# IQTLabs/WITW

Measured on AMD Instinct MI355X. Metric: image-pairs/sec (embedding+similarity), higher is better.
Workload: dtype f32

## Files before the change

include/witw_hip.h:

```cpp
#ifndef WITW_HIP_H
#define WITW_HIP_H

#ifdef __cplusplus
extern "C" {
#endif

const char* witw_last_error(void);
int witw_version(void);
int witw_device_check(int device);
const char* witw_last_kernel_variant(void);
const char* witw_last_conv_form(void);


int witw_conv3x3_tile_n(int cout);
int witw_conv3x3_workgroup_waves(int B, int H, int W, int Cout, int stride_h);
long long witw_conv3x3_packed_floats(int cout, int cin);
int witw_conv3x3_bias_floats(int cout);
int witw_conv3x3_pack_weights(const float* w_kcrs, float* wpk, int cout, int cin, int transpose_flip, void* stream);
int witw_nchw_to_nhwc8(const float* x, float* y, int B, int C, int H, int W, void* stream);
int witw_conv3x3_fwd(const float* x, const float* wpk, const float* bias, const float* dropmask, float* y, int B, int H,
                     int W, int Cin, int Cout, int stride_h, int pad_circular, int relu, int pool, int out_nchw,
                     void* stream);

int witw_conv3x3_first_pack(const float* w, float* wf, int C, int round_bf16, void* stream);
int witw_conv_first2_bf16_fwd(const float* x, const void* wf0, const float* bias0, const void* wpk2, const float* bias2, void* y,
                              int B, int C, int H, int W, int pad_circular, void* stream);
int witw_conv_first2_bf16_fwd_train(const float* x, const void* wf0, const float* bias0, const void* wpk2, const float* bias2, void* y,
                                    unsigned char* pool_code, unsigned char* gate_bits, int B, int C, int H, int W, int pad_circular,
                                    void* stream);
int witw_conv3x3_bf16_gatebits_ok(int B, int H, int W, int Cin, int Cout);
int witw_conv3x3_bf16_fwd_gatebits(const void* x_bf16, const void* wpk_bf16, const float* bias, const void* gate_bits, void* y, int B, int H,
                                   int W, int Cin, int Cout, int pad_circular, int relu, void* stream);
int witw_conv3x3_first_fwd(const float* x, const float* wf, const float* bias, void* y, int B, int C, int H, int W,
                           int pad_circular, int relu, int out_bf16, void* stream);

int witw_conv3x3_fwd_ex(const float* x, const float* wpk, const float* bias, const float* dropmask, const float* gate,
                        const float* post_scale, const float* post_shift, float* y, unsigned char* pool_code, int B, int H,
                        int W, int Cin, int Cout, int stride_h, int pad_circular, int relu, float lrelu_slope, int pool,
                        int out_nchw, int dilate_h, void* stream);
int witw_conv3x3_dil_skip(int enable);
long long witw_conv3x3_packed_floats_wino(int cout, int cin);
int witw_conv3x3_pack_weights_wino(const float* w_kcrs, float* wpk_wino, int cout, int cin, void* stream);
int witw_conv3x3_fwd_wino(const float* x, const float* wpk, const float* wpk_wino, const float* bias, const float* dropmask,
                          const float* gate, const float* post_scale, const float* post_shift, float* y, unsigned char* pool_code,
                          int B, int H, int W, int Cin, int Cout, int stride_h, int pad_circular, int relu, float lrelu_slope,
                          int pool, int out_nchw, int dilate_h, void* stream);
int witw_conv3x3_wino(int enable);
int witw_conv3x3_wino_run(int enable);
int witw_maxpool2x2_bwd(const float* dy, const unsigned char* pool_code, float* dx, int B, int Hp, int Wp, int H, int W,
                        int C, void* stream);
int witw_nchw_to_nhwc(const float* x, float* y, int B, int C, int H, int W, int Cpad, void* stream);
int witw_conv3x3_wgrad_splits(int B, int Ho, int Wo, int Cin, int Cout);
long long witw_conv3x3_wgrad_workspace_floats(int B, int H, int W, int Cin, int Cout, int stride_h);
int witw_conv3x3_wgrad(const float* x, const float* dz, float* dw, float* db, float* workspace, int B, int H, int W, int Cin,
                       int cin_real, int Cout, int stride_h, int pad_circular, int accumulate, void* stream);
int witw_adam_step(float* param, const float* grad, float* exp_avg, float* exp_avg_sq, long long n, float lr, float beta1,
                   float beta2, float eps, int step, void* stream);
int witw_adam_step_multi(float* const* param, const float* const* grad, float* const* exp_avg, float* const* exp_avg_sq,
                         const long long* n, const int* step, int count, float lr, float beta1, float beta2, float eps, void* stream);

long long witw_match_workspace_floats(int Bo, int Bs);
int witw_match_fwd(const float* ov, const float* su, int Bo, int Bs, int We, long long* orientation, float* distance,
                   float* score, float* workspace, void* stream);
int witw_match_fwd_masked(const float* ov, const float* su, int Bo, int Bs, int We, long long* orientation, float* distance,
                          float* score, float* workspace, const unsigned long long* shift_mask, void* stream);
long long witw_match_fixed_workspace_floats(int Bo, int Bs);
int witw_match_fwd_fixed(const float* ov, const float* su, int Bo, int Bs, int We, const long long* shift ,
                         long long* orientation, float* distance, float* score, float* workspace, void* stream);
long long witw_match_spectrum_floats(long long n_embeddings);
int witw_match_spectrum(const float* emb, float* spec, int B, int W, int role ,
                        void* stream);
long long witw_match_dft_workspace_floats(int Bo, int Bs);
int witw_match_fwd_dft(const float* ov, const float* su, const float* spec_ov, const float* spec_su, int Bo, int Bs, int We,
                       long long* orientation, float* distance, float* score, float* workspace, void* stream);
int witw_match_fwd_dft_gap(const float* ov, const float* su, const float* spec_ov, const float* spec_su, int Bo, int Bs, int We,
                           long long* orientation, float* distance, float* score, float* gap, float* workspace, void* stream);
int witw_match_fwd_dft_masked(const float* ov, const float* su, const float* spec_ov, const float* spec_su, int Bo, int Bs, int We,
                              long long* orientation, float* distance, float* score, float* gap , float* workspace,
                              const unsigned long long* shift_mask, void* stream);
long long witw_match_bwd_scratch_floats(int Bo, int Bs, int We);
int witw_match_bwd(const float* ov, const float* su, const long long* orientation, const float* score, const float* workspace,
                   const float* grad_distance, float* grad_ov, float* grad_su, float* scratch, int Bo, int Bs, int We,
                   void* stream);
int witw_crop_overhead(const float* ov, const long long* orientation, float* out , int Bo, int Bs,
                       int We, void* stream);
int witw_l2_distance(const float* cropped , const float* su , float* distance, int Bo, int Bs, int n,
                     void* stream);
int witw_rank_count(const float* distance , int* ranks , int Bo, int Bs, int true_offset, void* stream);

int witw_topk_smallest(const float* distance, float* values, long long* indices, int Bo, int Bs, int k, long long row_offset,
                       void* stream);
long long witw_topk_workspace_bytes(int Bo, int Bs, int k);
int witw_topk_smallest_ws(const float* distance, float* values, long long* indices, int Bo, int Bs, int k, long long row_offset,
                          void* workspace, void* stream);
int witw_topk_smallest_after(const float* distance, float* values, long long* indices, int Bo, int Bs, int k, long long row_offset,
                             const float* after_value, const long long* after_index, void* workspace, void* stream);
int witw_rank_count_thresh(const float* distance, const float* threshold, int* ranks, int Bo, int Bs, void* stream);

int witw_match_pairs(const float* ov, const float* su, const float* wn, const float* sn, const int* pair_o, const int* pair_s,
                     int n_pairs, int Bo, int Bs, int We, long long* orientation, float* distance, float* score, void* stream);
int witw_rank_count_band(const float* distance, const float* threshold, float eps, int* counts, int* pair_o, int* pair_s,
// ... 204 lines not shown
```

witw_amd/_lib.py:

```python
import ctypes
import os
from ctypes import c_char_p, c_float, c_int, c_longlong, c_void_p

from . import build as _build

_LIB = None
_GUARDS = None

SIGNATURES = {
    'witw_last_error': (c_char_p, []),
    'witw_version': (c_int, []),
    'witw_last_kernel_variant': (c_char_p, []),
    'witw_last_conv_form': (c_char_p, []),
    'witw_device_check': (c_int, [c_int]),
    'witw_conv3x3_tile_n': (c_int, [c_int]),
    'witw_conv3x3_workgroup_waves': (c_int, [c_int] * 5),
    'witw_conv3x3_packed_floats': (c_longlong, [c_int, c_int]),
    'witw_conv3x3_bias_floats': (c_int, [c_int]),
    'witw_conv3x3_pack_weights': (c_int, [c_void_p, c_void_p, c_int, c_int, c_int, c_void_p]),
    'witw_nchw_to_nhwc8': (c_int, [c_void_p, c_void_p, c_int, c_int, c_int, c_int, c_void_p]),
    'witw_conv3x3_fwd': (c_int, [c_void_p, c_void_p, c_void_p, c_void_p, c_void_p] + [c_int] * 10 + [c_void_p]),
    'witw_conv3x3_fwd_ex': (c_int, [c_void_p] * 9 + [c_int] * 8 + [c_float] + [c_int] * 3 + [c_void_p]),
    'witw_conv3x3_dil_skip': (c_int, [c_int]),
    'witw_conv3x3_packed_floats_wino': (c_longlong, [c_int, c_int]),
    'witw_conv3x3_pack_weights_wino': (c_int, [c_void_p, c_void_p, c_int, c_int, c_void_p]),
    'witw_conv3x3_fwd_wino': (c_int, [c_void_p] * 10 + [c_int] * 8 + [c_float] + [c_int] * 3 + [c_void_p]),
    'witw_conv3x3_wino': (c_int, [c_int]),
    'witw_conv3x3_wino_run': (c_int, [c_int]),
    'witw_maxpool2x2_bwd': (c_int, [c_void_p, c_void_p, c_void_p] + [c_int] * 6 + [c_void_p]),
    'witw_conv3x3_packed_floats_taps4': (c_longlong, [c_int, c_int]),
    'witw_conv3x3_pack_weights_taps4': (c_int, [c_void_p, c_void_p, c_int, c_int, c_int, c_void_p]),
    'witw_conv3x3_fwd_taps4': (c_int, [c_void_p] * 7 + [c_int] * 6 + [c_float, c_int, c_void_p]),
    'witw_conv3x3_taps4_ksplit': (c_int, [c_int] * 5),
    'witw_conv3x3_fwd_taps4_ex': (c_int, [c_void_p] * 7 + [c_int] * 6 + [c_float] + [c_int] * 5 + [c_void_p]),
    'witw_conv3x3_wgrad_taps4': (c_int, [c_void_p] * 5 + [c_int] * 7 + [c_void_p]),
    'witw_nchw_to_nhwc': (c_int, [c_void_p, c_void_p, c_int, c_int, c_int, c_int, c_int, c_void_p]),
    'witw_conv3x3_wgrad_splits': (c_int, [c_int] * 5),
    'witw_conv3x3_wgrad_workspace_floats': (c_longlong, [c_int] * 6),
    'witw_conv3x3_wgrad': (c_int, [c_void_p] * 5 + [c_int] * 9 + [c_void_p]),
    'witw_adam_step': (c_int, [c_void_p, c_void_p, c_void_p, c_void_p, c_longlong, c_float, c_float, c_float, c_float, c_int,
                               c_void_p]),
    'witw_adam_step_multi': (c_int, [c_void_p] * 6 + [c_int, c_float, c_float, c_float, c_float, c_void_p]),
    'witw_conv3x3_first_pack': (c_int, [c_void_p, c_void_p, c_int, c_int, c_void_p]),
    'witw_conv3x3_first_fwd': (c_int, [c_void_p, c_void_p, c_void_p, c_void_p] + [c_int] * 7 + [c_void_p]),
    'witw_conv3x3_bf16_mfma16': (c_int, [c_int]),
    'witw_conv3x3_bf16_wres': (c_int, [c_int]),
    'witw_conv3x3_bf16_packed_elems': (c_longlong, [c_int, c_int]),
    'witw_conv3x3_bf16_pack_weights': (c_int, [c_void_p, c_void_p, c_int, c_int, c_void_p]),
    'witw_conv3x3_bf16_pack_weights_ex': (c_int, [c_void_p, c_void_p, c_int, c_int, c_int, c_void_p]),
    'witw_conv3x3_bf16_pack_weights_multi': (c_int, [c_void_p] * 7 + [c_int, c_void_p]),
    'witw_nchw_f32_to_nhwc_bf16': (c_int, [c_void_p, c_void_p] + [c_int] * 5 + [c_void_p]),
    'witw_conv3x3_bf16_fwd': (c_int, [c_void_p] * 4 + [c_int] * 10 + [c_void_p]),
    'witw_conv3x3_bf16_fwd_ex': (c_int, [c_void_p] * 7 + [c_int] * 11 + [c_void_p]),
    'witw_maxpool2x2_bwd_bf16': (c_int, [c_void_p] * 3 + [c_int] * 6 + [c_void_p]),
    'witw_octet_elems': (c_longlong, [c_int] * 4),
    'witw_nhwc_bf16_to_octet': (c_int, [c_void_p, c_void_p] + [c_int] * 4 + [c_void_p]),
    'witw_conv3x3_wgrad_bf16_workspace_floats': (c_longlong, [c_int] * 6),
    'witw_conv3x3_wgrad_bf16': (c_int, [c_void_p] * 5 + [c_int] * 9 + [c_void_p]),
    'witw_conv3x3_wgrad_bf16_nhwc_workspace_floats': (c_longlong, [c_int] * 6),
    'witw_conv3x3_wgrad_bf16_mfma16': (c_int, [c_int]),
    'witw_conv3x3_wgrad_bf16_nhwc': (c_int, [c_void_p] * 5 + [c_int] * 9 + [c_void_p]),
    'witw_conv3x3_f16x3_packed_elems': (c_longlong, [c_int, c_int]),
    'witw_conv3x3_f16x3_pack_weights': (c_int, [c_void_p, c_void_p, c_int, c_int, c_void_p]),
    'witw_nchw_f32_to_split_f16': (c_int, [c_void_p, c_void_p] + [c_int] * 5 + [c_void_p]),
    'witw_split_f16_to_f32': (c_int, [c_void_p, c_void_p, c_longlong, c_int, c_void_p]),
    'witw_conv3x3_f16x3_fwd': (c_int, [c_void_p] * 4 + [c_int] * 10 + [c_void_p]),
    'witw_conv3x3_f16x3_pack_weights_ex': (c_int, [c_void_p, c_void_p, c_int, c_int, c_int, c_void_p]),
    'witw_conv3x3_f16x3_fwd_ex': (c_int, [c_void_p] * 8 + [c_int] * 11 + [c_void_p]),
    'witw_maxpool2x2_bwd_split': (c_int, [c_void_p] * 3 + [c_int] * 6 + [c_void_p]),
    'witw_octet_split_elems': (c_longlong, [c_int] * 4),
    'witw_split_f16_to_octet': (c_int, [c_void_p, c_void_p] + [c_int] * 4 + [c_void_p]),
    'witw_conv3x3_wgrad_f16x3_workspace_floats': (c_longlong, [c_int] * 6),
    'witw_conv3x3_wgrad_f16x3': (c_int, [c_void_p] * 6 + [c_int] * 9 + [c_void_p]),
    'witw_conv4x4s2_first_fwd': (c_int, [c_void_p] * 6 + [c_int] * 5 + [c_float, c_void_p]),
    'witw_conv4x4s2_first_fwd_bf16': (c_int, [c_void_p] * 6 + [c_int] * 5 + [c_float, c_void_p]),
    'witw_conv3x3_bf16_packed_elems_taps4': (c_longlong, [c_int, c_int]),
    'witw_conv3x3_bf16_pack_weights_taps4': (c_int, [c_void_p, c_void_p, c_int, c_int, c_void_p]),
    'witw_conv3x3_bf16_fwd_taps4': (c_int, [c_void_p] * 6 + [c_int] * 5 + [c_float] + [c_int] * 3 + [c_void_p]),
    'witw_conv3x3_bf16_taps4_ksplit': (c_int, [c_int] * 5),
    'witw_conv3x3_bf16_fwd_taps4_splitk': (c_int, [c_void_p] * 3 + [c_int] * 6 + [c_void_p]),
    'witw_space_to_depth2_mosaic_bf16': (c_int, [c_void_p, c_void_p] + [c_int] * 5 + [c_void_p]),
# ... 148 lines not shown
```

witw_amd/csrc/conv3x3.hip:

```cpp
#include "common.h"
#include <stdlib.h>
#include <algorithm>

namespace {

constexpr int TW_WIDE = 64;

__device__ const f32x4 g_zero_f4[1] = {{0.f, 0.f, 0.f, 0.f}};

struct ConvArgs {
    const float* x;
    const float* wpk;
    const float* bias;
    const float* dropmask;
    const float* post_scale;
    const float* post_shift;
    float lrelu;
    unsigned char* pool_code;
    const float* gate;
    float* y;
    int B, H, W, Cin, Cout;
    int Ho, Wo;
    int tiles_x, tiles_y;
    int n_tiles, sp_total, sp_per_xcd, xcd_map;
    int circ, relu, out_nchw;
    int force_nw;
    int force_geo;
    int dil_h;
    int tap_base;
    int ksplit, kc_per_split;
    size_t split_stride;
    int s2d, s2d_h, s2d_w, valid_h, valid_w;
    int wino;
    const float* wpk_wino;
    int wino_items, wino_wgs;
#ifdef WITW_STAMPS
    unsigned long long* stamps;
#endif
};

template <int NW, bool POOL>
__device__ __forceinline__ void conv_wino_h2(const ConvArgs& p, f32x4* smem) {
    constexpr int TH = NW, TW = 64, IW = TW + 2, IH = TH + 2;
    constexpr int NTHREADS = 64 * NW;
    constexpr int WTN = 64;
    constexpr int IN_F4 = 2 * IH * IW;
    constexpr int W_F4 = 12 * 2 * WTN;
    constexpr int STAGE_F4 = IN_F4 + W_F4;
    constexpr int NIN = (IN_F4 + NTHREADS - 1) / NTHREADS;
    constexpr int NWT = W_F4 / NTHREADS;
    static_assert(NWT * NTHREADS == W_F4, "the filter slab splits evenly over the workgroup");

    int tid = threadIdx.x;
    asm volatile("" : "+v"(tid));
    const int lane = tid & 63;
    const int wave = tid >> 6;
    const int l31 = lane & 31;
    const int hq = lane >> 5;

    const int tiles_img = p.tiles_x * p.tiles_y;
    auto item_sp = [&](int it, int& ntile) {
        if (p.xcd_map) {
            const int g = it >> 3;
            ntile = g % p.n_tiles;
            return (it & 7) * p.sp_per_xcd + g / p.n_tiles;
        }
        ntile = it / p.sp_total;
        return it - ntile * p.sp_total;
    };
    auto step_item = [&](int it) { return p.wino_items - it > p.wino_wgs ? it + p.wino_wgs : p.wino_items; };
    auto next_item = [&](int it) {
        int nt;
        while (it < p.wino_items && item_sp(it, nt) >= p.sp_total) it = step_item(it);
        return it;
    };
    int it = next_item(blockIdx.x);
    if (it >= p.wino_items) return;
    const int nkc = p.Cin >> 3;

    constexpr unsigned OOR = 0x80000000u;
    const size_t img_floats = (size_t)p.H * p.W * p.Cin;
    int ntile, b, oy0, ox0;
    __amdgpu_buffer_rsrc_t in_rs, w_rs;
    unsigned gin[NIN];
    auto decode = [&](int item, int& nt_, int& b_, int& oy0_, int& ox0_) {
        int sp = item_sp(item, nt_);
        b_ = sp / tiles_img;
        sp -= b_ * tiles_img;
        const int ty = sp / p.tiles_x;
        oy0_ = ty * TH;
        ox0_ = (sp - ty * p.tiles_x) * TW;
    };
    auto stage_from = [&](int nt_, int b_, int oy0_, int ox0_, bool live) {
        in_rs = __builtin_amdgcn_make_buffer_rsrc((void*)(p.x + (size_t)b_ * img_floats), 0, live ? (unsigned)(img_floats * 4) : 0u,
                                                  0x00020000);
        w_rs = __builtin_amdgcn_make_buffer_rsrc((void*)(reinterpret_cast<const f32x4*>(p.wpk_wino) + (size_t)nt_ * nkc * W_F4), 0,
                                                 live ? (unsigned)nkc * W_F4 * 16u : 0u, 0x00020000);
        if (!live) return;
        int t = tid;
        asm volatile("" : "+v"(t));
#pragma unroll
        for (int i = 0; i < NIN; ++i) {
            const int s = t + i * NTHREADS;
            const int pix = s >> 1, q = s & 1;
            const int r = pix / IW, c = pix - r * IW;
            const int gr = oy0_ - 1 + r;
            int gc = ox0_ - 1 + c;
            bool ok = (s < IN_F4) && gr >= 0 && gr < p.H;
            if (p.circ) {
                gc %= p.W;
                if (gc < 0) gc += p.W;
            } else {
                ok = ok && gc >= 0 && gc < p.W;
            }
            gin[i] = ok ? (unsigned)((((size_t)gr * p.W + gc) * p.Cin + q * 4) * 4) : OOR;
        }
    };
    decode(it, ntile, b, oy0, ox0);
    stage_from(ntile, b, oy0, ox0, true);
    const unsigned gwoff = (unsigned)tid * 16u;
    f32x4 rin[NIN], rw[NWT];
    auto load_one = [&](int kc, int i) {
        if (i < NIN) rin[i] = __builtin_bit_cast(f32x4, __builtin_amdgcn_raw_buffer_load_b128(in_rs, gin[i], (unsigned)kc * 32u, 0));
        else rw[i - NIN] = __builtin_bit_cast(f32x4, __builtin_amdgcn_raw_buffer_load_b128(
                 w_rs, gwoff, (unsigned)kc * W_F4 * 16u + (unsigned)(i - NIN) * (NTHREADS * 16u), 0));
    };
    auto store_one = [&](int buf, int i) {
        f32x4* in_s = smem + buf * STAGE_F4;
        if (i < NIN) {
            const int s = tid + i * NTHREADS;
            f32x4* dst = (NIN * NTHREADS == IN_F4 || s < IN_F4) ? in_s + (s & 1) * (IH * IW) + (s >> 1) : smem + 2 * STAGE_F4;
            *dst = rin[i];
        } else {
            in_s[IN_F4 + tid + (i - NIN) * NTHREADS] = rw[i - NIN];
        }
    };

    const int wm = wave >> 1, wn = wave & 1;
    const int abase = hq * (IH * IW) + 2 * wm * IW + l31;
    const int wbase = hq * WTN + wn * 32 + l31;
    f32x16 acc[4][2];
#pragma unroll
    for (int t = 0; t < 4; ++t)
#pragma unroll
        for (int ct = 0; ct < 2; ++ct)
#pragma unroll
            for (int r = 0; r < 16; ++r) acc[t][ct][r] = 0.f;

    f32x4 fa[2][4], fb[2][4];
    auto read_a = [&](int set, const f32x4* in_s, int s, int i) { fa[set][i] = in_s[abase + i * IW + 32 * (s & 1) + (s >> 1)]; };
    auto read_b = [&](int set, const f32x4* w_s, int kw, int t) { fb[set][t] = w_s[(kw * 4 + t) * 2 * WTN + wbase]; };
    auto transform2 = [&](int set, int k) {
        const int j = k >> 1;
        const float d0 = fa[set][0][j], d1 = fa[set][1][j], d2 = fa[set][2][j], d3 = fa[set][3][j];
        if ((k & 1) == 0) {
            fa[set][0][j] = d0 - d2;
            fa[set][3][j] = d1 - d3;
        } else {
            fa[set][1][j] = d1 + d2;
            fa[set][2][j] = d2 - d1;
        }
    };
    auto mfma_one = [&](int set, int bset, int ct, int i) {
        const int j = i >> 2, t = i & 3;
        acc[t][ct] = __builtin_amdgcn_mfma_f32_32x32x2f32(fa[set][t][j], fb[bset][t][j], acc[t][ct], 0, 0, 0);
    };

#pragma unroll
    for (int i = 0; i < NIN + NWT; ++i) load_one(0, i);
#pragma unroll
    for (int i = 0; i < NIN + NWT; ++i) store_one(0, i);
    __syncthreads();
#pragma unroll
    for (int i = 0; i < 4; ++i) read_b(0, smem + IN_F4, 0, i);
    __builtin_amdgcn_sched_barrier(0);
#pragma unroll
    for (int i = 0; i < 4; ++i) read_a(0, smem, 0, i);
#pragma unroll
    for (int k = 0; k < 8; ++k) transform2(0, k);

    auto step = [&](int set, int bset, int ct, auto&& mem, bool barrier_mid) {
#pragma unroll
        for (int i = 0; i < 16; ++i) {
            mfma_one(set, bset, ct, i);
            mem(i);
            if (i >= 8) transform2(set ^ 1, i - 8);
            __builtin_amdgcn_sched_barrier(0);
            if (barrier_mid && i == 7) {
                __syncthreads();
                __builtin_amdgcn_sched_barrier(0);
            }
        }
    };
    static_assert(16 - 6 - (NIN + NWT) >= 0, "step too short to hide the staging instructions");

    auto chunk = [&](int cur, int kn) __attribute__((always_inline)) {
        const f32x4* in_s = smem + cur * STAGE_F4;
        const f32x4* w_s = in_s + IN_F4;
        const f32x4* in_n = smem + (cur ^ 1) * STAGE_F4;
        step(0, 0, 0, [&](int i) {
            if (i < 4) read_a(1, in_s, 1, i);
            else if (i < 6) read_b(1, w_s, 1, i - 4);
            else if (i < 6 + NIN + NWT) load_one(kn, i - 6);
        }, false);
        step(1, 0, 1, [&](int i) {
            if (i < 4) read_a(0, in_s, 2, i);
            else if (i < 6) read_b(1, w_s, 1, i - 2);
        }, false);
        step(0, 1, 0, [&](int i) {
            if (i < 4) read_a(1, in_s, 3, i);
            else if (i < 8) read_b(0, w_s, 2, i - 4);
        }, false);
        step(1, 1, 1, [&](int i) {
            if (i < 4) read_a(0, in_s, 4, i);
            else if (i < 4 + NIN + NWT) store_one(cur ^ 1, i - 4);
        }, false);
        step(0, 0, 0, [&](int i) {
            if (i < 4) read_a(1, in_s, 5, i);
        }, true);
        step(1, 0, 1, [&](int i) {
            if (i < 4) read_a(0, in_n, 0, i);
            else if (i < 8) read_b(1, in_n + IN_F4, 0, i - 4);
        }, false);
#pragma unroll
        for (int t = 0; t < 4; ++t) fb[0][t] = fb[1][t];
    };

    const int Hy = POOL ? (p.Ho >> 1) : p.Ho;
    const int Wy = POOL ? (p.Wo >> 1) : p.Wo;
    float* slab = reinterpret_cast<float*>(smem + 2 * STAGE_F4 + 1) + wave * (32 * 32);
    const int prow = lane >> 3, pc4 = (lane & 7) * 4;
    int cur = 0;
    for (;;) {
        for (int kc = 1; kc < nkc; ++kc) {
            chunk(cur, kc);
            cur ^= 1;
        }
        const int it_n = next_item(step_item(it));
        const bool more = it_n < p.wino_items;
        int ntile_n = ntile, b_n = b, oy0_n = oy0, ox0_n = ox0;
        if (more) decode(it_n, ntile_n, b_n, oy0_n, ox0_n);
        stage_from(ntile_n, b_n, oy0_n, ox0_n, more);
        chunk(cur, 0);
        cur ^= 1;

        const int n0 = ntile * WTN;
        f32x16 yv[2][2];
#pragma unroll
        for (int ct = 0; ct < 2; ++ct)
#pragma unroll
            for (int r = 0; r < 16; ++r) {
                const float m0 = acc[0][ct][r], m1 = acc[1][ct][r], m2 = acc[2][ct][r], m3 = acc[3][ct][r];
                yv[0][ct][r] = (m0 + m1) + m2;
                yv[1][ct][r] = (m1 - m2) - m3;
            }
        const int nb = n0 + wn * 32;
        const int nch = nb + l31;
        const float bv = p.bias[nch];
        const float dm = (p.dropmask != nullptr && nch < p.Cout) ? p.dropmask[(size_t)b * p.Cout + nch] : 1.f;
        const int act = p.relu;
        auto fin = [&](float v) {
            v = (v + bv) * dm;
            if (act == 1) v = fmaxf(v, 0.f);
            else if (act == 2) v = v > 0.f ? v : v * p.lrelu;
            return v;
        };
        if constexpr (!POOL) {
#pragma unroll
            for (int k = 0; k < 2; ++k)
#pragma unroll
                for (int ct = 0; ct < 2; ++ct) {
#pragma unroll
                    for (int r = 0; r < 16; ++r) slab[((r & 3) + 8 * (r >> 2) + 4 * hq) * 32 + l31] = fin(yv[k][ct][r]);
                    const int yy = oy0 + 2 * wm + k;
#pragma unroll
// ... 19 lines not shown
                        const int pc = 16 * ct + 4 * g + 2 * hq + e;
                        slab[pc * 32 + l31] = fin(m);
                        const int xx = (ox0 >> 1) + pc;
                        if (p.pool_code != nullptr && yy < Hy && xx < Wy && nch < p.Cout) {
                            const int code = (a00 == m) ? 0 : (a01 == m) ? 1 : (a10 == m) ? 2 : 3;
                            p.pool_code[(((size_t)b * Hy + yy) * Wy + xx) * p.Cout + nch] = (unsigned char)code;
                        }
                    }
#pragma unroll
            for (int g = 0; g < 4; ++g) {
                const int pc = g * 8 + prow;
                const f32x4 v = *reinterpret_cast<const f32x4*>(slab + pc * 32 + pc4);
                const int xx = (ox0 >> 1) + pc;
                if (yy < Hy && xx < Wy && nb + pc4 < p.Cout)
                    __builtin_nontemporal_store(v, reinterpret_cast<f32x4*>(p.y + (((size_t)b * Hy + yy) * Wy + xx) * p.Cout + nb + pc4));
            }
        }
        if (!more) break;
        it = it_n;
        ntile = ntile_n;
        b = b_n;
        oy0 = oy0_n;
        ox0 = ox0_n;
#pragma unroll
        for (int t = 0; t < 4; ++t)
#pragma unroll
            for (int ct = 0; ct < 2; ++ct)
#pragma unroll
                for (int r = 0; r < 16; ++r) acc[t][ct][r] = 0.f;
    }
}

template <int TN, int SH, bool POOL, int NW, int GEO, int TAPS = 9>
__global__ __launch_bounds__(64 * NW) void conv3x3_nhwc_f32_kernel(ConvArgs p) {
    static_assert(TAPS == 9 || TAPS == 4, "3x3 window or a 2x2 sub-window");
    constexpr bool NARROW = GEO == 1;
    constexpr bool DIL = GEO == 2;
    static_assert(!DIL || (TN == 128 && NW == 8 && SH == 1 && TAPS == 9 && !POOL), "the dilated form exists for the 8-wave 128-channel tile");
    constexpr int TH = NARROW ? 4 * NW : NW;
    constexpr int TW = NARROW ? 16 : 64;
    constexpr int IW = TW + 2;
    constexpr int NTHREADS = 64 * NW;
    constexpr int IH = (TH - 1) * SH + 3;
    constexpr int IN_F4 = 2 * IH * IW;
    constexpr int W_F4 = TAPS * 2 * TN;
    constexpr int STAGE_F4 = IN_F4 + W_F4;
    constexpr int NIN = (IN_F4 + NTHREADS - 1) / NTHREADS;
    constexpr int NWT = (W_F4 + NTHREADS - 1) / NTHREADS;
    constexpr int WGM = (TN == 128) ? NW / 2 : NW;
    constexpr int WM = (2 * NW) / WGM;
    constexpr int WN = 2;

    constexpr bool WINO = SH == 1 && TAPS == 9 && GEO == 0 && (TN == 128 || POOL);
    constexpr int WINO_F4 = WINO ? 2 * (2 * (NW + 2) * IW + 12 * 2 * 64) + 1 + NW * 256 : 0;
    constexpr int DIRECT_F4 = (2 * STAGE_F4 + 1 > NW * 512) ? 2 * STAGE_F4 + 1 : NW * 512;
    constexpr int SMEM_F4 = DIRECT_F4 > WINO_F4 ? DIRECT_F4 : WINO_F4;
    __shared__ f32x4 smem[SMEM_F4];
    static_assert(SMEM_F4 * 16 >= NW * 32 * 64 * 4, "the buffer must hold one epilogue slab per wave");
    if constexpr (WINO) {
        if (__builtin_expect(p.wino != 0, 0)) {
            conv_wino_h2<NW, POOL>(p, smem);
            return;
        }
    }

    const int tid = threadIdx.x;
    const int lane = tid & 63;
    const int wave = tid >> 6;
    const int l31 = lane & 31;
    const int hq = lane >> 5;

    int ntile, sp;
    if (p.xcd_map) {
        const int g = blockIdx.x >> 3;
        ntile = g % p.n_tiles;
        sp = (blockIdx.x & 7) * p.sp_per_xcd + g / p.n_tiles;
        if (sp >= p.sp_total) return;
    } else {
        ntile = blockIdx.x / p.sp_total;
        sp = blockIdx.x - ntile * p.sp_total;
    }
    const int tiles_img = p.tiles_x * p.tiles_y;
    const int b = sp / tiles_img;
    sp -= b * tiles_img;
    const int ty = sp / p.tiles_x;
    const int tx = sp - ty * p.tiles_x;
    const int oy0 = ty * TH;
    const int ox0 = tx * TW;
    const int n0 = ntile * TN;
    int nkc = p.Cin >> 3;
    int kc_lo = 0;
    if constexpr (TAPS == 4) {
        if (p.ksplit > 1) {
            kc_lo = (int)blockIdx.y * p.kc_per_split;
            nkc = min(nkc - kc_lo, p.kc_per_split);
        }
    }

    constexpr unsigned OOR = 0x80000000u;
    const int Hp = p.dil_h ? (p.H - 1) / 2 + 1 : p.H;
    const size_t img_floats = (size_t)Hp * p.W * p.Cin;
    __amdgpu_buffer_rsrc_t in_rs = __builtin_amdgcn_make_buffer_rsrc(
        (void*)(p.x + (size_t)b * img_floats + (size_t)kc_lo * 8), 0, (unsigned)(img_floats * 4) - (unsigned)kc_lo * 32u, 0x00020000);
    const unsigned wtile_bytes = (unsigned)nkc * W_F4 * 16u;
    __amdgpu_buffer_rsrc_t w_rs = __builtin_amdgcn_make_buffer_rsrc(
        (void*)(reinterpret_cast<const f32x4*>(p.wpk) + ((size_t)ntile * (p.Cin >> 3) + kc_lo) * W_F4), 0, wtile_bytes, 0x00020000);
    unsigned gin[NIN];
#pragma unroll
    for (int i = 0; i < NIN; ++i) {
        const int s = tid + i * NTHREADS;
        const int pix = s >> 1, q = s & 1;
        const int r = pix / IW, c = pix - r * IW;
        const int gr = oy0 * SH - 1 + r;
        int gc = ox0 - 1 + c;
// ... 420 lines not shown
    }
    reinterpret_cast<f32x4*>(wpk)[idx] = v;
}

__global__ void pack_weights_wino_kernel(const float* __restrict__ w, float* __restrict__ wpk, int Cout, int Cin, int nkc,
                                         size_t total) {
    const size_t idx = (size_t)blockIdx.x * blockDim.x + threadIdx.x;
    if (idx >= total) return;
    size_t t = idx;
    const int n = t % 64; t /= 64;
    const int q = t % 2; t /= 2;
    const int tr = t % 4; t /= 4;
    const int kw = t % 3; t /= 3;
    const int kc = t % nkc; t /= nkc;
    const int co = (int)t * 64 + n;
    f32x4 v = {0.f, 0.f, 0.f, 0.f};
#pragma unroll
    for (int j = 0; j < 4; ++j) {
        const int ci = kc * 8 + q * 4 + j;
        if (co < Cout && ci < Cin) {
            const float* g = w + ((size_t)co * Cin + ci) * 9 + kw;
            const float g0 = g[0], g1 = g[3], g2 = g[6];
            v[j] = tr == 0 ? g0 : tr == 1 ? ((g0 + g1) + g2) * 0.5f : tr == 2 ? ((g0 - g1) + g2) * 0.5f : g2;
        }
    }
    reinterpret_cast<f32x4*>(wpk)[idx] = v;
}

__global__ void nchw_to_nhwc8_kernel(const float* __restrict__ x, float* __restrict__ y, int B, int C, int H, int W) {
    const size_t npix = (size_t)B * H * W;
    const size_t idx = (size_t)blockIdx.x * blockDim.x + threadIdx.x;
    if (idx >= npix) return;
    const size_t hw = (size_t)H * W;
    const size_t b = idx / hw, r = idx - b * hw;
    float v[8];
#pragma unroll
    for (int c = 0; c < 8; ++c) v[c] = (c < C) ? x[(b * C + c) * hw + r] : 0.f;
    f32x4* o = reinterpret_cast<f32x4*>(y + idx * 8);
    o[0] = f32x4{v[0], v[1], v[2], v[3]};
    o[1] = f32x4{v[4], v[5], v[6], v[7]};
}

__global__ void nchw_to_nhwc_kernel(const float* __restrict__ x, float* __restrict__ y, int C, int Cp, size_t hw, size_t total) {
    const size_t idx = (size_t)blockIdx.x * blockDim.x + threadIdx.x;
    if (idx >= total) return;
    const int c = idx % Cp;
    const size_t t = idx / Cp;
    const size_t b = t / hw, r = t - b * hw;
    y[idx] = (c < C) ? x[(b * C + c) * hw + r] : 0.f;
}

int env_int(const char* name, int dflt);
int wino_run();

template <int TN, int SH, bool POOL, int NW, int GEO, int TAPS = 9>
int launch_conv_nw(ConvArgs a, hipStream_t st) {
    a.tiles_y = cdiv(a.Ho, GEO == 1 ? 4 * NW : NW);
    a.tiles_x = cdiv(a.Wo, GEO == 1 ? 16 : 64);
    const long long sp_total = (long long)a.B * a.tiles_x * a.tiles_y;
    a.n_tiles = cdiv(a.Cout, a.wino ? 64 : TN);
    a.sp_per_xcd = (int)((sp_total + 7) / 8);
    if (sp_total < 8) a.xcd_map = 0;
    const long long grid = a.xcd_map ? 8LL * a.sp_per_xcd * a.n_tiles : sp_total * a.n_tiles;
    if (grid <= 0 || grid > 0x7fffffffLL || sp_total > 0x7fffffffLL) {
        witw_set_error("conv3x3: grid %lld out of range", grid);
        return WITW_ERR_INVALID;
    }
    a.sp_total = (int)sp_total;
    const unsigned gy = (TAPS == 4 && a.ksplit > 1) ? (unsigned)a.ksplit : 1u;
    a.wino_items = (int)grid;
    a.wino_wgs = (int)grid;
    if (a.wino && wino_run()) {
        const int forced = env_int("WITW_CONV_WINO_WGS", 0);
        a.wino_wgs = (int)std::min<long long>(grid, forced > 0 ? forced : witw_cu_count());
    }
    hipLaunchKernelGGL((conv3x3_nhwc_f32_kernel<TN, SH, POOL, NW, GEO, TAPS>), dim3(a.wino ? (unsigned)a.wino_wgs : (unsigned)grid, gy),
                       dim3(64 * NW), 0, st, a);
    WITW_CHECK_LAUNCH("conv3x3_nhwc_f32");
    witw_note_variant("conv3x3_nhwc_f32_kernel<%d,%d,%s,%d,%d,%d>", TN, SH, POOL ? "true" : "false", NW, GEO, TAPS);
    if (a.wino) witw_note_conv_form("wino_h2");
    return WITW_OK;
}

int choose_waves(int B, int Ho, int Wo, int Cout, int force_nw) {
    const int TN = (Cout >= 128) ? 128 : 64;
    const long long big = (long long)cdiv(Cout, TN) * B * cdiv(Wo, TW_WIDE) * cdiv(Ho, 8);
    if (force_nw == 4) return 4;
    return (force_nw == 8 || ((Ho % 8) == 0 && witw_fills_rounds(big))) ? 8 : 4;
}

bool choose_narrow(int Wo, int force_geo) { return force_geo == 1 || (force_geo != 0 && Wo <= 32); }

int env_int(const char* name, int dflt) {
    const char* e = getenv(name);
    return e ? atoi(e) : dflt;
}

int g_dil_skip = -1;
int dil_skip() {
    if (g_dil_skip < 0) {
        const char* e = getenv("WITW_CONV_DILSKIP");
        g_dil_skip = e ? (atoi(e) != 0) : 1;
    }
    return g_dil_skip;
}

int g_wino = -1;
int wino_on() {
    if (g_wino < 0) {
        const char* e = getenv("WITW_CONV_WINO");
        g_wino = e ? (atoi(e) != 0) : 1;
    }
    return g_wino;
}

int g_wino_run = -1;
int wino_run() {
    if (g_wino_run < 0) {
        const char* e = getenv("WITW_CONV_WINO_RUN");
        g_wino_run = e ? (atoi(e) != 0) : 1;
    }
    return g_wino_run;
}

template <int TN, int SH, bool POOL>
int launch_conv(ConvArgs a, hipStream_t st) {
    const bool wino = SH == 1 && (TN == 128 || POOL) && a.wpk_wino != nullptr && wino_on() && a.gate == nullptr && !a.dil_h &&
                      !a.out_nchw && a.post_scale == nullptr && (a.Cout & 3) == 0 && a.force_geo != 1 &&
                      !choose_narrow(a.Wo, a.force_geo);
    a.wino = wino ? 1 : 0;
    if (wino) return choose_waves(a.B, a.Ho, a.Wo, a.Cout, a.force_nw) == 8 ? launch_conv_nw<TN, SH, POOL, 8, 0>(a, st)
                                                                          : launch_conv_nw<TN, SH, POOL, 4, 0>(a, st);
#ifndef WITW_NO_NARROW
    if (choose_narrow(a.Wo, a.force_geo)) return launch_conv_nw<TN, SH, POOL, 4, 1>(a, st);
#endif
    if (choose_waves(a.B, a.Ho, a.Wo, a.Cout, a.force_nw) == 8) {
        if constexpr (TN == 128 && SH == 1 && !POOL) {
            if (a.dil_h && dil_skip()) return launch_conv_nw<TN, SH, POOL, 8, 2>(a, st);
        }
        return launch_conv_nw<TN, SH, POOL, 8, 0>(a, st);
    }
    return launch_conv_nw<TN, SH, POOL, 4, 0>(a, st);
}

template <int TN>
int launch_conv_taps4(const ConvArgs& a, hipStream_t st) {
#ifndef WITW_NO_NARROW
    if (choose_narrow(a.Wo, a.force_geo)) return launch_conv_nw<TN, 1, false, 4, 1, 4>(a, st);
#endif
    if (choose_waves(a.B, a.Ho, a.Wo, a.Cout, a.force_nw) == 8) return launch_conv_nw<TN, 1, false, 8, 0, 4>(a, st);
    return launch_conv_nw<TN, 1, false, 4, 0, 4>(a, st);
}

}

#ifdef WITW_STAMPS
unsigned long long* witw_conv_stamps_ptr = nullptr;
#endif

extern "C" {

int witw_conv3x3_tile_n(int cout) { return cout >= 128 ? 128 : 64; }

int witw_conv3x3_workgroup_waves(int B, int H, int W, int Cout, int stride_h) {
    if (B <= 0 || H <= 0 || W <= 0 || Cout <= 0 || (stride_h != 1 && stride_h != 2)) return -1;
    if (choose_narrow(W, env_int("WITW_CONV_GEO", -1))) return 4;
    return choose_waves(B, (H + 2 - 3) / stride_h + 1, W, Cout, env_int("WITW_CONV_NW", 0));
}

long long witw_conv3x3_packed_floats(int cout, int cin) {
    if (cout <= 0 || cin <= 0) return -1;
    const int TN = witw_conv3x3_tile_n(cout);
    const long long n_tiles = cdiv(cout, TN), nkc = cdiv(cin, 8);
    return n_tiles * nkc * 9 * 2 * TN * 4;
}
// ... 159 lines not shown
    a.tiles_y = 0;
    a.force_nw = env_int("WITW_CONV_NW", 0);
    a.force_geo = env_int("WITW_CONV_GEO", -1);
    a.xcd_map = env_int("WITW_CONV_XCD", 1) != 0;
    a.circ = pad_circular; a.relu = relu; a.out_nchw = out_nchw; a.dil_h = dilate_h; a.tap_base = 0;
    a.ksplit = 1; a.kc_per_split = 0; a.split_stride = 0; a.s2d = 0; a.s2d_h = a.s2d_w = a.valid_h = a.valid_w = 0;
    a.wino = 0; a.wpk_wino = wpk_wino;
#ifdef WITW_STAMPS
    a.stamps = witw_conv_stamps_ptr;
#endif
    hipStream_t st = (hipStream_t)stream;
    const int TN = witw_conv3x3_tile_n(Cout);
    if (TN == 128) {
        if (stride_h == 2) return launch_conv<128, 2, false>(a, st);
        return pool ? launch_conv<128, 1, true>(a, st) : launch_conv<128, 1, false>(a, st);
    }
    if (stride_h == 2) return launch_conv<64, 2, false>(a, st);
    return pool ? launch_conv<64, 1, true>(a, st) : launch_conv<64, 1, false>(a, st);
}

}

extern "C" {

int witw_conv3x3_fwd_ex(const float* x, const float* wpk, const float* bias, const float* dropmask, const float* gate,
                        const float* post_scale, const float* post_shift, float* y, unsigned char* pool_code, int B, int H,
                        int W, int Cin, int Cout, int stride_h, int pad_circular, int relu, float lrelu_slope, int pool,
                        int out_nchw, int dilate_h, void* stream) {
    return conv3x3_fwd_any(x, wpk, nullptr, bias, dropmask, gate, post_scale, post_shift, y, pool_code, B, H, W, Cin, Cout,
                           stride_h, pad_circular, relu, lrelu_slope, pool, out_nchw, dilate_h, stream);
}

int witw_conv3x3_fwd_wino(const float* x, const float* wpk, const float* wpk_wino, const float* bias, const float* dropmask,
                          const float* gate, const float* post_scale, const float* post_shift, float* y, unsigned char* pool_code,
                          int B, int H, int W, int Cin, int Cout, int stride_h, int pad_circular, int relu, float lrelu_slope,
                          int pool, int out_nchw, int dilate_h, void* stream) {
    WITW_CHECK_ARG(wpk_wino, "conv3x3_fwd_wino: null Winograd filter");
    return conv3x3_fwd_any(x, wpk, wpk_wino, bias, dropmask, gate, post_scale, post_shift, y, pool_code, B, H, W, Cin, Cout,
                           stride_h, pad_circular, relu, lrelu_slope, pool, out_nchw, dilate_h, stream);
}

int witw_conv3x3_wino(int enable) {
    const int prev = wino_on();
    if (enable >= 0) g_wino = enable != 0;
    return prev;
}

int witw_conv3x3_wino_run(int enable) {
    const int prev = wino_run();
    if (enable >= 0) g_wino_run = enable != 0;
    return prev;
}

long long witw_conv3x3_packed_floats_wino(int cout, int cin) {
    if (cout <= 0 || cin <= 0) return -1;
    return (long long)cdiv(cout, 64) * cdiv(cin, 8) * 12 * 2 * 64 * 4;
}

int witw_conv3x3_pack_weights_wino(const float* w_kcrs, float* wpk_wino, int cout, int cin, void* stream) {
    WITW_CHECK_ARG(w_kcrs && wpk_wino, "pack_weights_wino: null pointer");
    WITW_CHECK_ARG(cout > 0 && cin > 0, "pack_weights_wino: bad shape cout=%d cin=%d", cout, cin);
    const int n_tiles = cdiv(cout, 64), nkc = cdiv(cin, 8);
    const size_t total = (size_t)n_tiles * nkc * 12 * 2 * 64;
    hipLaunchKernelGGL(pack_weights_wino_kernel, dim3((unsigned)((total + 255) / 256)), dim3(256), 0, (hipStream_t)stream,
                       w_kcrs, wpk_wino, cout, cin, nkc, total);
    WITW_CHECK_LAUNCH("pack_weights_wino");
    return WITW_OK;
}

int witw_conv3x3_dil_skip(int enable) {
    const int prev = dil_skip();
    if (enable >= 0) g_dil_skip = enable != 0;
    return prev;
}

int witw_conv3x3_fwd(const float* x, const float* wpk, const float* bias, const float* dropmask, float* y, int B, int H,
                     int W, int Cin, int Cout, int stride_h, int pad_circular, int relu, int pool, int out_nchw,
                     void* stream) {
    return witw_conv3x3_fwd_ex(x, wpk, bias, dropmask, nullptr, nullptr, nullptr, y, nullptr, B, H, W, Cin, Cout, stride_h,
                               pad_circular, relu ? 1 : 0, 0.f, pool, out_nchw, 0, stream);
}

}
```

witw_amd/ops.py:

```python
import torch

from . import _lib


PROFILE = None
PROFILE_BY_KERNEL = None


def _stream():
    return torch.cuda.current_stream().cuda_stream


def _dev_f32(t, name):
    if not (isinstance(t, torch.Tensor) and t.is_cuda):
        raise _lib.WitwError('%s must be a CUDA(HIP) tensor: the WITW hot path has no CPU fallback' % name)
    if t.dtype != torch.float32:
        raise _lib.WitwError('%s must be float32, got %s' % (name, t.dtype))
    if not t.is_contiguous():
        raise _lib.WitwError('%s must be contiguous' % name)
    return t


def _p(t):
    return 0 if t is None else t.data_ptr()
# ... 1215 lines not shown

def gem_pool(x_nhwc, valid_hw, out, col0, p=3., scale=None, shift=None):
    lib = _lib.load()
    x = _dev_f32(x_nhwc, 'x')
    B, Hp, Wp, C = x.shape
    H, W = valid_hw
    _lib.check(lib.witw_gem_pool(x.data_ptr(), out.data_ptr(), B, Hp, Wp, H, W, C, out.shape[1], col0, float(p), _p(scale),
                                 _p(shift), _stream()), 'witw_gem_pool')
    return out


def embed_normalize_(f):
    lib = _lib.load()
    f = _dev_f32(f, 'f')
    _lib.check(lib.witw_embed_normalize(f.data_ptr(), f.shape[0], f.shape[1], _stream()), 'witw_embed_normalize')
    return f


def pairwise_sqdist(a, b, take_sqrt=False):
    lib = _lib.load()
    a, b = _dev_f32(a, 'a'), _dev_f32(b, 'b')
    if a.dim() != 2 or b.dim() != 2 or a.shape[1] != b.shape[1]:
        raise _lib.WitwError('pairwise_sqdist: need [Na,n] and [Nb,n]')
    D = torch.empty((a.shape[0], b.shape[0]), dtype=torch.float32, device=a.device)
    _lib.check(lib.witw_pairwise_sqdist(a.data_ptr(), b.data_ptr(), D.data_ptr(), a.shape[0], b.shape[0], a.shape[1],
                                        int(take_sqrt), _stream()), 'witw_pairwise_sqdist')
    return D


def exhaustive_triplet_loss(D, soft_margin=False, alpha=10., margin=1.):
    lib = _lib.load()
    D = _dev_f32(D, 'D')
    B = D.shape[0]
    loss = torch.empty((1,), dtype=torch.float32, device=D.device)
    ws = torch.empty((B,), dtype=torch.float32, device=D.device)
    _lib.check(lib.witw_exhaustive_triplet_loss(D.data_ptr(), B, int(soft_margin), float(alpha), float(margin),
                                                loss.data_ptr(), ws.data_ptr(), _stream()), 'witw_exhaustive_triplet_loss')
    return loss.reshape(())


def last_conv_form():
    v = _lib.load().witw_last_conv_form()
    return v.decode() if v else ''


def conv_wino(enable=None):
    return bool(_lib.load().witw_conv3x3_wino(-1 if enable is None else int(bool(enable))))


def conv_wino_run(enable=None):
    return bool(_lib.load().witw_conv3x3_wino_run(-1 if enable is None else int(bool(enable))))


def last_kernel_variant():
    v = _lib.load().witw_last_kernel_variant()
    return v.decode() if v else ''


def bf16_mfma16(enable=None):
    return bool(_lib.load().witw_conv3x3_bf16_mfma16(-1 if enable is None else int(bool(enable))))


def bf16_wres(enable=None):
    return bool(_lib.load().witw_conv3x3_bf16_wres(-1 if enable is None else int(bool(enable))))


class PackedConvBf16(_Packed):
    CPAD, DTYPE = 16, torch.bfloat16

    def __init__(self, weight, bias, transpose_flip=False, reuse=None):
        lib = _lib.load()
        w, reuse = self._filter_buffer(weight, transpose_flip, reuse, lib.witw_conv3x3_bf16_packed_elems)
        _lib.check(lib.witw_conv3x3_bf16_pack_weights_ex(w.data_ptr(), self.wpk.data_ptr(), self.cout, self.cin,
                                                         int(bool(transpose_flip)), _stream()), 'witw_conv3x3_bf16_pack_weights_ex')
        self._bias_buffer(reuse, bias)

    @classmethod
    def batch(cls, items):
        import ctypes
        lib = _lib.load()
        out, tab = [], []
        for weight, bias, transpose_flip, reuse in items:
            pk = cls.__new__(cls)
            w, reuse = pk._filter_buffer(weight, transpose_flip, reuse, lib.witw_conv3x3_bf16_packed_elems)
            pk._bias_buffer(reuse)
            b = None if bias is None else _dev_f32(bias.detach(), 'bias')
            if b is not None and b.numel() != pk.cout:
                raise _lib.WitwError('PackedConvBf16.batch: bias of %d elements for %d output channels' % (b.numel(), pk.cout))
            tab.append((w, pk.wpk, b, pk.bias, pk.cout, pk.cin, int(bool(transpose_flip))))
            out.append(pk)
        k = len(tab)
        if k:
            vp = ctypes.c_void_p
            _lib.check(lib.witw_conv3x3_bf16_pack_weights_multi(
                (vp * k)(*[t[0].data_ptr() for t in tab]), (vp * k)(*[t[1].data_ptr() for t in tab]),
                (vp * k)(*[None if t[2] is None else t[2].data_ptr() for t in tab]), (vp * k)(*[t[3].data_ptr() for t in tab]),
                (ctypes.c_int * k)(*[t[4] for t in tab]), (ctypes.c_int * k)(*[t[5] for t in tab]),
                (ctypes.c_int * k)(*[t[6] for t in tab]), k, _stream()), 'witw_conv3x3_bf16_pack_weights_multi')
        return out


def nchw_to_nhwc_bf16(x, cpad=16):
    lib = _lib.load()
    x = _dev_f32(x, 'x')
    B, C, H, W = x.shape
    y = torch.empty((B, H, W, cpad), dtype=torch.bfloat16, device=x.device)
# ... 291 lines not shown
```

Baseline: 2530.

## Stage Winograd conv inputs and filters via direct global-to-LDS buffer loads

Adds a DMA variant of the Winograd conv kernel that uses buffer loads writing straight into LDS instead of loading into registers and then storing to shared memory. The next chunk's transfers are spread over the MFMA steps, with a vmcnt wait before the mid barrier. The input staging layout is padded and reordered, plane-major instead of interleaved, to suit wave-contiguous LDS writes. It is on by default behind an env toggle. This saves registers and VALU/LDS store instructions, but it changes the LDS layout and how synchronisation is ordered.

```diff
diff --git a/include/witw_hip.h b/include/witw_hip.h
--- a/include/witw_hip.h
+++ b/include/witw_hip.h
@@ -47,6 +47,7 @@
                           int pool, int out_nchw, int dilate_h, void* stream);
 int witw_conv3x3_wino(int enable);
 int witw_conv3x3_wino_run(int enable);
+int witw_conv3x3_wino_dma(int enable);
 int witw_maxpool2x2_bwd(const float* dy, const unsigned char* pool_code, float* dx, int B, int Hp, int Wp, int H, int W,
                         int C, void* stream);
 int witw_nchw_to_nhwc(const float* x, float* y, int B, int C, int H, int W, int Cpad, void* stream);
diff --git a/witw_amd/_lib.py b/witw_amd/_lib.py
--- a/witw_amd/_lib.py
+++ b/witw_amd/_lib.py
@@ -27,6 +27,7 @@
     'witw_conv3x3_fwd_wino': (c_int, [c_void_p] * 10 + [c_int] * 8 + [c_float] + [c_int] * 3 + [c_void_p]),
     'witw_conv3x3_wino': (c_int, [c_int]),
     'witw_conv3x3_wino_run': (c_int, [c_int]),
+    'witw_conv3x3_wino_dma': (c_int, [c_int]),
     'witw_maxpool2x2_bwd': (c_int, [c_void_p, c_void_p, c_void_p] + [c_int] * 6 + [c_void_p]),
     'witw_conv3x3_packed_floats_taps4': (c_longlong, [c_int, c_int]),
     'witw_conv3x3_pack_weights_taps4': (c_int, [c_void_p, c_void_p, c_int, c_int, c_int, c_void_p]),
diff --git a/witw_amd/csrc/conv3x3.hip b/witw_amd/csrc/conv3x3.hip
--- a/witw_amd/csrc/conv3x3.hip
+++ b/witw_amd/csrc/conv3x3.hip
@@ -1,4 +1,5 @@
 #include "common.h"
+#include "lds_frag.h"
 #include <stdlib.h>
 #include <algorithm>
 
@@ -34,21 +35,23 @@
     int wino;
     const float* wpk_wino;
     int wino_items, wino_wgs;
+    int wino_dma;
 #ifdef WITW_STAMPS
     unsigned long long* stamps;
 #endif
 };
 
-template <int NW, bool POOL>
+template <int NW, bool POOL, bool DMA>
 __device__ __forceinline__ void conv_wino_h2(const ConvArgs& p, f32x4* smem) {
     constexpr int TH = NW, TW = 64, IW = TW + 2, IH = TH + 2;
     constexpr int NTHREADS = 64 * NW;
     constexpr int WTN = 64;
     constexpr int IN_F4 = 2 * IH * IW;
     constexpr int W_F4 = 12 * 2 * WTN;
-    constexpr int STAGE_F4 = IN_F4 + W_F4;
     constexpr int NIN = (IN_F4 + NTHREADS - 1) / NTHREADS;
     constexpr int NWT = W_F4 / NTHREADS;
+    constexpr int IN_PAD = NIN * NTHREADS;
+    constexpr int STAGE_F4 = IN_PAD + W_F4;
     static_assert(NWT * NTHREADS == W_F4, "the filter slab splits evenly over the workgroup");
 
     int tid = threadIdx.x;
@@ -82,6 +85,7 @@
     const size_t img_floats = (size_t)p.H * p.W * p.Cin;
     int ntile, b, oy0, ox0;
     __amdgpu_buffer_rsrc_t in_rs, w_rs;
+    i32x4 in_rd, w_rd;
     unsigned gin[NIN];
     auto decode = [&](int item, int& nt_, int& b_, int& oy0_, int& ox0_) {
         int sp = item_sp(item, nt_);
@@ -92,17 +96,24 @@
         ox0_ = (sp - ty * p.tiles_x) * TW;
     };
     auto stage_from = [&](int nt_, int b_, int oy0_, int ox0_, bool live) {
-        in_rs = __builtin_amdgcn_make_buffer_rsrc((void*)(p.x + (size_t)b_ * img_floats), 0, live ? (unsigned)(img_floats * 4) : 0u,
-                                                  0x00020000);
-        w_rs = __builtin_amdgcn_make_buffer_rsrc((void*)(reinterpret_cast<const f32x4*>(p.wpk_wino) + (size_t)nt_ * nkc * W_F4), 0,
-                                                 live ? (unsigned)nkc * W_F4 * 16u : 0u, 0x00020000);
+        const float* in_base = p.x + (size_t)b_ * img_floats;
+        const f32x4* w_base = reinterpret_cast<const f32x4*>(p.wpk_wino) + (size_t)nt_ * nkc * W_F4;
+        const unsigned in_bytes = live ? (unsigned)(img_floats * 4) : 0u, w_bytes = live ? (unsigned)nkc * W_F4 * 16u : 0u;
+        if constexpr (DMA) {
+            in_rd = raw_rsrc(in_base, in_bytes);
+            w_rd = raw_rsrc(w_base, w_bytes);
+        } else {
+            in_rs = __builtin_amdgcn_make_buffer_rsrc((void*)in_base, 0, in_bytes, 0x00020000);
+            w_rs = __builtin_amdgcn_make_buffer_rsrc((void*)w_base, 0, w_bytes, 0x00020000);
+        }
         if (!live) return;
         int t = tid;
         asm volatile("" : "+v"(t));
 #pragma unroll
         for (int i = 0; i < NIN; ++i) {
             const int s = t + i * NTHREADS;
-            const int pix = s >> 1, q = s & 1;
+            const int q = DMA ? (s >= IH * IW) : (s & 1);
+            const int pix = DMA ? s - q * (IH * IW) : s >> 1;
             const int r = pix / IW, c = pix - r * IW;
             const int gr = oy0_ - 1 + r;
             int gc = ox0_ - 1 + c;
@@ -119,6 +130,14 @@
     decode(it, ntile, b, oy0, ox0);
     stage_from(ntile, b, oy0, ox0, true);
     const unsigned gwoff = (unsigned)tid * 16u;
+    const unsigned smem_lds = (unsigned)__builtin_amdgcn_readfirstlane((int)lds_address(smem));
+    const unsigned wave_lds = (unsigned)__builtin_amdgcn_readfirstlane(wave) * 1024u;
+    auto dma_one = [&](int buf, int kc, int i) {
+        const unsigned st = smem_lds + (unsigned)buf * (STAGE_F4 * 16u) + wave_lds;
+        if (i < NIN) dma16(in_rd, st + (unsigned)i * (NTHREADS * 16u), gin[i], (unsigned)kc * 32u);
+        else dma16(w_rd, st + (unsigned)(IN_PAD + (i - NIN) * NTHREADS) * 16u, gwoff,
+                   (unsigned)kc * W_F4 * 16u + (unsigned)(i - NIN) * (NTHREADS * 16u));
+    };
     f32x4 rin[NIN], rw[NWT];
     auto load_one = [&](int kc, int i) {
         if (i < NIN) rin[i] = __builtin_bit_cast(f32x4, __builtin_amdgcn_raw_buffer_load_b128(in_rs, gin[i], (unsigned)kc * 32u, 0));
@@ -132,7 +151,7 @@
             f32x4* dst = (NIN * NTHREADS == IN_F4 || s < IN_F4) ? in_s + (s & 1) * (IH * IW) + (s >> 1) : smem + 2 * STAGE_F4;
             *dst = rin[i];
         } else {
-            in_s[IN_F4 + tid + (i - NIN) * NTHREADS] = rw[i - NIN];
+            in_s[IN_PAD + tid + (i - NIN) * NTHREADS] = rw[i - NIN];
         }
     };
 
@@ -166,13 +185,19 @@
         acc[t][ct] = __builtin_amdgcn_mfma_f32_32x32x2f32(fa[set][t][j], fb[bset][t][j], acc[t][ct], 0, 0, 0);
     };
 
-#pragma unroll
-    for (int i = 0; i < NIN + NWT; ++i) load_one(0, i);
-#pragma unroll
-    for (int i = 0; i < NIN + NWT; ++i) store_one(0, i);
+    if constexpr (DMA) {
+#pragma unroll
+        for (int i = 0; i < NIN + NWT; ++i) dma_one(0, 0, i);
+        wait_vmcnt<0>();
+    } else {
+#pragma unroll
+        for (int i = 0; i < NIN + NWT; ++i) load_one(0, i);
+#pragma unroll
+        for (int i = 0; i < NIN + NWT; ++i) store_one(0, i);
+    }
     __syncthreads();
 #pragma unroll
-    for (int i = 0; i < 4; ++i) read_b(0, smem + IN_F4, 0, i);
+    for (int i = 0; i < 4; ++i) read_b(0, smem + IN_PAD, 0, i);
     __builtin_amdgcn_sched_barrier(0);
 #pragma unroll
     for (int i = 0; i < 4; ++i) read_a(0, smem, 0, i);
@@ -187,6 +212,7 @@
             if (i >= 8) transform2(set ^ 1, i - 8);
             __builtin_amdgcn_sched_barrier(0);
             if (barrier_mid && i == 7) {
+                if constexpr (DMA) wait_vmcnt<0>();
                 __syncthreads();
                 __builtin_amdgcn_sched_barrier(0);
             }
@@ -196,31 +222,40 @@
 
     auto chunk = [&](int cur, int kn) __attribute__((always_inline)) {
         const f32x4* in_s = smem + cur * STAGE_F4;
-        const f32x4* w_s = in_s + IN_F4;
+        const f32x4* w_s = in_s + IN_PAD;
         const f32x4* in_n = smem + (cur ^ 1) * STAGE_F4;
+        constexpr int PER = (NIN + NWT + 2) / 3;
+        auto dma_gap = [&](int s, int i) {
+            const int j = s * PER + (i - 6);
+            if (i >= 6 && i < 6 + PER && j < NIN + NWT) dma_one(cur ^ 1, kn, j);
+        };
         step(0, 0, 0, [&](int i) {
             if (i < 4) read_a(1, in_s, 1, i);
             else if (i < 6) read_b(1, w_s, 1, i - 4);
+            else if (DMA) dma_gap(0, i);
             else if (i < 6 + NIN + NWT) load_one(kn, i - 6);
         }, false);
         step(1, 0, 1, [&](int i) {
             if (i < 4) read_a(0, in_s, 2, i);
             else if (i < 6) read_b(1, w_s, 1, i - 2);
+            else if (DMA) dma_gap(1, i);
         }, false);
         step(0, 1, 0, [&](int i) {
             if (i < 4) read_a(1, in_s, 3, i);
-            else if (i < 8) read_b(0, w_s, 2, i - 4);
+            else if (i < (DMA ? 6 : 8)) read_b(0, w_s, 2, i - 4);
+            else if (DMA) dma_gap(2, i);
         }, false);
         step(1, 1, 1, [&](int i) {
             if (i < 4) read_a(0, in_s, 4, i);
-            else if (i < 4 + NIN + NWT) store_one(cur ^ 1, i - 4);
+            else if (DMA && i < 6) read_b(0, w_s, 2, i - 2);
+            else if (!DMA && i < 4 + NIN + NWT) store_one(cur ^ 1, i - 4);
         }, false);
         step(0, 0, 0, [&](int i) {
             if (i < 4) read_a(1, in_s, 5, i);
         }, true);
         step(1, 0, 1, [&](int i) {
             if (i < 4) read_a(0, in_n, 0, i);
-            else if (i < 8) read_b(1, in_n + IN_F4, 0, i - 4);
+            else if (i < 8) read_b(1, in_n + IN_PAD, 0, i - 4);
         }, false);
 #pragma unroll
         for (int t = 0; t < 4; ++t) fb[0][t] = fb[1][t];
@@ -346,14 +381,16 @@
     constexpr int WN = 2;
 
     constexpr bool WINO = SH == 1 && TAPS == 9 && GEO == 0 && (TN == 128 || POOL);
-    constexpr int WINO_F4 = WINO ? 2 * (2 * (NW + 2) * IW + 12 * 2 * 64) + 1 + NW * 256 : 0;
+    constexpr int WINO_IN_F4 = (2 * (NW + 2) * IW + NTHREADS - 1) / NTHREADS * NTHREADS;
+    constexpr int WINO_F4 = WINO ? 2 * (WINO_IN_F4 + 12 * 2 * 64) + 1 + NW * 256 : 0;
     constexpr int DIRECT_F4 = (2 * STAGE_F4 + 1 > NW * 512) ? 2 * STAGE_F4 + 1 : NW * 512;
     constexpr int SMEM_F4 = DIRECT_F4 > WINO_F4 ? DIRECT_F4 : WINO_F4;
     __shared__ f32x4 smem[SMEM_F4];
     static_assert(SMEM_F4 * 16 >= NW * 32 * 64 * 4, "the buffer must hold one epilogue slab per wave");
     if constexpr (WINO) {
         if (__builtin_expect(p.wino != 0, 0)) {
-            conv_wino_h2<NW, POOL>(p, smem);
+            if (p.wino_dma) conv_wino_h2<NW, POOL, true>(p, smem);
+            else conv_wino_h2<NW, POOL, false>(p, smem);
             return;
         }
     }
@@ -880,6 +917,7 @@
 
 int env_int(const char* name, int dflt);
 int wino_run();
+int wino_dma();
 
 template <int TN, int SH, bool POOL, int NW, int GEO, int TAPS = 9>
 int launch_conv_nw(ConvArgs a, hipStream_t st) {
@@ -902,6 +940,7 @@
         const int forced = env_int("WITW_CONV_WINO_WGS", 0);
         a.wino_wgs = (int)std::min<long long>(grid, forced > 0 ? forced : witw_cu_count());
     }
+    a.wino_dma = a.wino ? wino_dma() : 0;
     hipLaunchKernelGGL((conv3x3_nhwc_f32_kernel<TN, SH, POOL, NW, GEO, TAPS>), dim3(a.wino ? (unsigned)a.wino_wgs : (unsigned)grid, gy),
                        dim3(64 * NW), 0, st, a);
     WITW_CHECK_LAUNCH("conv3x3_nhwc_f32");
@@ -949,6 +988,15 @@
         g_wino_run = e ? (atoi(e) != 0) : 1;
     }
     return g_wino_run;
+}
+
+int g_wino_dma = -1;
+int wino_dma() {
+    if (g_wino_dma < 0) {
+        const char* e = getenv("WITW_CONV_WINO_DMA");
+        g_wino_dma = e ? (atoi(e) != 0) : 1;
+    }
+    return g_wino_dma;
 }
 
 template <int TN, int SH, bool POOL>
@@ -1214,6 +1262,12 @@
     return prev;
 }
 
+int witw_conv3x3_wino_dma(int enable) {
+    const int prev = wino_dma();
+    if (enable >= 0) g_wino_dma = enable != 0;
+    return prev;
+}
+
 long long witw_conv3x3_packed_floats_wino(int cout, int cin) {
     if (cout <= 0 || cin <= 0) return -1;
     return (long long)cdiv(cout, 64) * cdiv(cin, 8) * 12 * 2 * 64 * 4;
diff --git a/witw_amd/ops.py b/witw_amd/ops.py
--- a/witw_amd/ops.py
+++ b/witw_amd/ops.py
@@ -1291,6 +1291,10 @@
     return bool(_lib.load().witw_conv3x3_wino_run(-1 if enable is None else int(bool(enable))))
 
 
+def conv_wino_dma(enable=None):
+    return bool(_lib.load().witw_conv3x3_wino_dma(-1 if enable is None else int(bool(enable))))
+
+
 def last_kernel_variant():
     v = _lib.load().witw_last_kernel_variant()
     return v.decode() if v else ''
```

Result: faster. 2600, median of 6 (+2.8%).
